# junyongeom/gru-mpi-cuda

Hardware: AMD Instinct MI355X
Metric: char-tokens/sec (whole node) for GRU hidden=512 at 1/2/4/8 MI355X (higher is better)
Workload: dtype bf16; 1 GPU; model=GRU L=1 H=512 E=512 V=256, global_batch=256, seq_len=32, parallelism=dp1, impl=hip, optimizer=adam, overlap=False, plan=fwd=persistent bwd0=persistent+dWhh+dP head=fwd-tail serial dP=bwd-tail, dp_plan=replicated, dp_pipeline=0, collectives=0

## Files before the change

### gru_mpi_cuda_amd/csrc/bindings.cpp

```cpp
#include <pybind11/pybind11.h>
#include <pybind11/numpy.h>
#include <pybind11/stl.h>

#include "engine/trainer.h"
#include "engine/generator.h"
#include "comm/rccl_comm.h"
#include "comm/bootstrap.h"
#include "data/name_loader.h"

namespace py = pybind11;
using namespace gk;

static hipStream_t S(uintptr_t s) { return reinterpret_cast<hipStream_t>(s); }
template <class T> static T* Pp(uintptr_t p) { return reinterpret_cast<T*>(p); }

template <class T>
static T get(const py::dict& d, const char* k, T dflt) {
  if (!d.contains(k)) return dflt;
  return d[k].cast<T>();
}
#define GP(T, d, k) reinterpret_cast<T*>(get<uintptr_t>(d, k, 0))

static OptimArgs optim_from(const py::dict& d, const std::string& who) {
  OptimArgs a;
// ... 367 lines not shown
  m.def("adam_step", [](py::dict o, uintptr_t s) {
    const OptimArgs a = optim_from(o, "adam_step");
    if (!a.g) throw std::runtime_error("adam_step: g required");
    adam_step(a, S(s));
    HIP_LAUNCH_CHECK();
  });
  m.def("grad_clip_scale", [](py::dict d, uintptr_t s) {
    const float* x = GP(const float, d, "x");
    float* parts = GP(float, d, "parts");
    float* scale = GP(float, d, "scale");
    const long n = get<long>(d, "n", 0);
    const int nparts = get<int>(d, "nparts", 0);
    if (!x || !parts || !scale || n < 0 || nparts < 1 || nparts > 4096)
      throw std::runtime_error("grad_clip_scale: x, parts, scale, n >= 0 and 1 <= nparts <= 4096 required");
    sumsq_partials(x, n, parts, nparts, S(s));
    HIP_LAUNCH_CHECK();
    clip_scale_finalize(parts, nparts, get<float>(d, "clip", 0.f), scale, S(s));
    HIP_LAUNCH_CHECK();
  });
  m.def("reduce_slabs_multi", [](py::list jobs, uintptr_t bump, uintptr_t s) {
    SlabJobs j;
    if (jobs.size() > 24) throw std::runtime_error("reduce_slabs_multi: at most 24 jobs");
    if (jobs.size() == 0) throw std::runtime_error("reduce_slabs_multi: no jobs");
    for (auto h : jobs) {
      py::dict d = h.cast<py::dict>();
      const float* src = GP(const float, d, "src");
      const int splits = get<int>(d, "splits", 1);
      if (!src || splits < 1) throw std::runtime_error("reduce_slabs_multi: src and splits >= 1 required");
      if (d.contains("bf") || d.contains("bfT") || d.contains("R") || d.contains("C")) {
        const int R = get<int>(d, "R", 0), C = get<int>(d, "C", 0);
        if (!GP(u16, d, "bf") && !GP(u16, d, "bfT")) throw std::runtime_error("reduce_slabs_multi: cast job needs bf or bfT");
        if (R <= 0 || C <= 0) throw std::runtime_error("reduce_slabs_multi: cast job needs R, C > 0");
        j.add_cast(src, splits, R, C, GP(float, d, "dst"), GP(u16, d, "bf"), GP(u16, d, "bfT"));
      } else {
        const long n = get<long>(d, "n", 0);
        if (n < 1 || !GP(float, d, "dst")) throw std::runtime_error("reduce_slabs_multi: plain job needs n >= 1 and dst");
        j.add(src, splits, n, GP(float, d, "dst"));
      }
    }
    j.bump = Pp<int>(bump);
    reduce_slabs_multi(j, S(s));
    HIP_LAUNCH_CHECK();
  });
  m.def("sum_partials", [](uintptr_t parts, int n, uintptr_t out, uintptr_t bump, uintptr_t s) {
    if (!parts || !out || n < 0) throw std::runtime_error("sum_partials: parts, out and n >= 0 required");
    sum_partials(Pp<const float>(parts), n, Pp<float>(out), S(s), Pp<int>(bump));
    HIP_LAUNCH_CHECK();
  });
  m.def("flat_pack_u32", [](uintptr_t p, uintptr_t pack, std::vector<std::pair<long, long>> ranges, long lo, long hi,
                            long tail, int unpack, uintptr_t s) {
    if (ranges.size() > 16) throw std::runtime_error("flat_pack_u32: at most 16 ranges");
    if (!p || !pack) throw std::runtime_error("flat_pack_u32: p and pack required");
    FlatRanges r;
    for (const auto& [off, n] : ranges) {
      if (off < 0 || n < 0 || n > (1L << 30)) throw std::runtime_error("flat_pack_u32: bad range");
      r.off[r.cnt] = off;
      r.n[r.cnt++] = (int)n;
    }
    flat_pack_u32(Pp<float>(p), Pp<unsigned>(pack), r, lo, hi, tail, unpack, S(s));
    HIP_LAUNCH_CHECK();
  });
  auto fwd_step_args = [](py::dict d) {
    FwdStepArgs a;
    a.hprev_bf = GP(const u16, d, "hprev_bf"); a.hprev_f = GP(const float, d, "hprev_f");
    a.Whh = GP(const u16, d, "Whh"); a.bhh = GP(const float, d, "bhh");
    a.P = GP(const float, d, "P"); a.ids = GP(const int, d, "ids"); a.Gi = GP(const float, d, "Gi");
    a.x_bf = GP(const u16, d, "x_bf"); a.Wih = GP(const u16, d, "Wih"); a.bih = GP(const float, d, "bih");
    a.Kin = get<int>(d, "Kin", 0);
    a.h_f = GP(float, d, "h_f"); a.h_bf = GP(u16, d, "h_bf"); a.hT = GP(u16, d, "hT");
    a.ldT = get<int>(d, "ldT", 0); a.colT = get<int>(d, "colT", 0);
    a.sr = GP(float, d, "sr"); a.sz = GP(float, d, "sz"); a.sn = GP(float, d, "sn"); a.sghn = GP(float, d, "sghn");
    a.s16 = GP(u16, d, "s16");
    a.Bp = get<int>(d, "Bp", 0); a.H = get<int>(d, "H", 0); a.algo = get<int>(d, "algo", 0);
    if (a.Bp % 32 || a.H % 64) throw std::runtime_error("fwd_step: Bp % 32 and H % 64 required");
    return a;
  };
  auto bwd_step_args = [](py::dict d) {
    BwdStepArgs a;
    a.dgh_next = GP(const u16, d, "dgh_next"); a.WhhT = GP(const u16, d, "WhhT");
    a.carry_in = GP(const float, d, "carry_in"); a.dy = GP(const float, d, "dy");
    a.r = GP(const float, d, "r"); a.z = GP(const float, d, "z"); a.n = GP(const float, d, "n");
    a.ghn = GP(const float, d, "ghn"); a.hprev = GP(const float, d, "hprev");
    a.carry_out = GP(float, d, "carry_out"); a.dgh = GP(u16, d, "dgh"); a.dghT = GP(u16, d, "dghT");
    a.dgiT = GP(u16, d, "dgiT"); a.dgi = GP(u16, d, "dgi");
    a.ldT = get<int>(d, "ldT", 0); a.colT = get<int>(d, "colT", 0);
    a.Bp = get<int>(d, "Bp", 0); a.H = get<int>(d, "H", 0); a.algo = get<int>(d, "algo", 0);
    a.sk_part = GP(float, d, "sk_part"); a.sk_part_floats = get<long>(d, "sk_part_floats", 0);
    a.sk_cnt = GP(unsigned, d, "sk_cnt"); a.sk_cnt_words = get<long>(d, "sk_cnt_words", 0);
    a.err = GP(unsigned, d, "err");
    a.dgiT_n_only = get<int>(d, "dgiT_n_only", 0);
    if (a.Bp % 32 || a.H % 64) throw std::runtime_error("bwd_step: Bp % 32 and H % 64 required");
    return a;
  };
  m.def("fwd_step", [fwd_step_args](py::dict d, uintptr_t s) {
    gru_fwd_step(fwd_step_args(d), S(s));
    HIP_LAUNCH_CHECK();
  });
  m.def("bwd_step", [bwd_step_args](py::dict d, uintptr_t s) {
    gru_bwd_step(bwd_step_args(d), S(s));
    HIP_LAUNCH_CHECK();
  });
  auto plan_dict = [](const StepPlan& p) {
    py::dict o;
    o["name"] = step_kernel_name(p.kernel);
    o["ks"] = p.ks; o["kb"] = p.kb; o["nks_i"] = p.nks_i; o["splits"] = p.splits; o["sk_map"] = p.sk_map;
    return o;
  };
  m.def("fwd_step_variant", [fwd_step_args, plan_dict](py::dict d) { return plan_dict(gru_fwd_step_plan(fwd_step_args(d))); });
  m.def("bwd_step_variant", [bwd_step_args, plan_dict](py::dict d) { return plan_dict(gru_bwd_step_plan(bwd_step_args(d))); });
  m.def("spin_delay", [](int us, uintptr_t s) { spin_delay(us, S(s)); HIP_LAUNCH_CHECK(); });
  m.def("copy_d2d", [](uintptr_t dst, uintptr_t src, size_t bytes) {
    HIP_CHECK(hipMemcpy(reinterpret_cast<void*>(dst), reinterpret_cast<const void*>(src), bytes, hipMemcpyDeviceToDevice));
  });
  m.def("graph_node_probe_detail", &graph_node_probe_detail);
  m.def("graph_node_probe", &graph_node_probe);
  m.def("block_cus", [](int nblocks, int us, uintptr_t s) { block_cus(nblocks, us, S(s)); });
  m.def("xcc_census", [](uintptr_t out, int nblocks, int threads, uintptr_t s) {
    xcc_census(Pp<unsigned>(out), nblocks, threads, S(s)); HIP_LAUNCH_CHECK(); });
  m.def("fwd_seq_supported", &gru_fwd_seq_supported);
  m.def("bwd_step_sk_splits", &gru_bwd_step_sk_splits);
  m.def("step_lds_variants", []() {
    const StepLdsVariants& v = step_lds_variants();
    py::dict d;
    d["fwd64"] = v.fwd64; d["bwd_sk_min_h"] = v.bwd_sk_min_h; d["dwfc_group"] = v.dwfc_group;
    d["bwd_big"] = v.bwd_big; d["bwd16"] = v.bwd16; d["bwd_xring"] = v.bwd_xring; d["fwd_xring"] = v.fwd_xring; d["fwd_fc"] = v.fwd_fc; d["fc_flash"] = v.fc_flash; d["fc_tail"] = v.fc_tail; d["bwd_tail"] = v.bwd_tail; d["save16"] = v.save16; d["big_dy"] = v.big_dy; d["ld_pad"] = v.ld_pad;
    return d;
  });
  m.def("set_step_lds_variants", [](py::dict d) {
    StepLdsVariants& v = step_lds_variants();
    for (auto kv : d) {
      const std::string k = py::str(kv.first);
      const int x = kv.second.cast<int>();
      if (k == "fwd64") v.fwd64 = x;
      else if (k == "bwd_sk_min_h") v.bwd_sk_min_h = x;
      else if (k == "dwfc_group") v.dwfc_group = x;
      else if (k == "bwd_big") v.bwd_big = x;
      else if (k == "bwd16") v.bwd16 = x;
      else if (k == "bwd_xring") v.bwd_xring = x;
      else if (k == "fwd_xring") v.fwd_xring = x;
      else if (k == "fwd_fc") v.fwd_fc = x;
      else if (k == "fc_flash") v.fc_flash = x;
      else if (k == "fc_tail") v.fc_tail = x;
      else if (k == "bwd_tail") v.bwd_tail = x;
      else if (k == "big_dy") v.big_dy = x;
      else if (k == "ld_pad") v.ld_pad = x;
      else if (k == "save16") v.save16 = x;
      else throw std::runtime_error("set_step_lds_variants: unknown field " + k);
    }
  });
  m.def("gemm_variants", []() {
    const GemmVariants& v = gemm_variants();
    py::dict d;
    d["mfma"] = v.mfma; d["phased"] = v.phased; d["sched"] = v.sched; d["groupm"] = v.groupm; d["onehot"] = v.onehot;
    return d;
  });
  m.def("set_gemm_variants", [](py::dict d) {
    GemmVariants& v = gemm_variants();
    for (auto kv : d) {
      const std::string k = py::str(kv.first);
      const int x = kv.second.cast<int>();
      if (k == "mfma") v.mfma = x;
      else if (k == "phased") v.phased = x;
      else if (k == "sched") v.sched = x;
      else if (k == "groupm") v.groupm = x;
      else if (k == "onehot") v.onehot = x;
      else throw std::runtime_error("set_gemm_variants: unknown field " + k);
    }
  });
  m.def("bwd_seq_supported", &gru_bwd_seq_supported);
  m.def("fwd_seq2", [](py::dict lo, py::dict hi, uintptr_t Wih, uintptr_t bih, uintptr_t s) {
    auto parse = [](py::dict d) {
      SeqFwdArgs a;
      a.HSb = GP(u16, d, "HSb"); a.HSf = GP(float, d, "HSf"); a.HT = GP(u16, d, "HT"); a.ldT = get<int>(d, "ldT", 0);
      a.HF = GP(u16, d, "HF"); a.xch = GP(u16, d, "xch");
      a.sr = GP(float, d, "sr"); a.sz = GP(float, d, "sz"); a.sn = GP(float, d, "sn"); a.sghn = GP(float, d, "sghn");
      a.Whh = GP(const u16, d, "Whh"); a.bhh = GP(const float, d, "bhh");
      a.P = GP(const float, d, "P"); a.ids = GP(const int, d, "ids"); a.Gi = GP(const float, d, "Gi");
      a.h0 = GP(const float, d, "h0");
      a.cnt = GP(unsigned, d, "cnt"); a.err = GP(unsigned, d, "err");
      a.dbg = GP(unsigned long long, d, "dbg"); a.allow_local = get<int>(d, "allow_local", 1);
      a.xring = get<int>(d, "xring", 0);
      a.s16 = GP(u16, d, "s16");
      a.zero_next = GP(unsigned, d, "zero_next"); a.zero_words = get<long>(d, "zero_words", 0);
      a.T = get<int>(d, "T", 0); a.Bp = get<int>(d, "Bp", 0); a.H = get<int>(d, "H", 0);
      if (!a.xch || !a.cnt || !a.HSb || !a.HSf || !a.Whh || !a.bhh) throw std::runtime_error("fwd_seq2: HSb/HSf/xch/cnt/Whh/bhh required");
      return a;
    };
    SeqFwd2Args a;
    a.lo = parse(lo); a.hi = parse(hi);
    a.Wih = reinterpret_cast<const u16*>(Wih); a.bih = reinterpret_cast<const float*>(bih);
    if (!a.lo.ids == !a.lo.Gi) throw std::runtime_error("fwd_seq2: lo needs exactly one of P+ids / Gi");
    if (!gru_fwd_seq2_supported(a.lo.H, a.lo.Bp)) throw std::runtime_error("fwd_seq2: shape not supported");
    gru_fwd_seq2(a, S(s));
    HIP_LAUNCH_CHECK();
  });
  m.def("fwd_seq2_supported", &gru_fwd_seq2_supported);
  m.def("fwd_seq_fc_supported", &gru_fwd_seq_fc_supported);
  m.def("fwd_seq_fc", [](py::dict d, py::dict fd, uintptr_t s) {
    SeqFwdArgs a;
    a.HSb = GP(u16, d, "HSb"); a.HSf = GP(float, d, "HSf"); a.HT = GP(u16, d, "HT"); a.ldT = get<int>(d, "ldT", 0);
    a.HF = GP(u16, d, "HF"); a.xch = GP(u16, d, "xch");
    a.sr = GP(float, d, "sr"); a.sz = GP(float, d, "sz"); a.sn = GP(float, d, "sn"); a.sghn = GP(float, d, "sghn");
    a.Whh = GP(const u16, d, "Whh"); a.bhh = GP(const float, d, "bhh");
    a.P = GP(const float, d, "P"); a.ids = GP(const int, d, "ids"); a.Gi = GP(const float, d, "Gi");
    a.h0 = GP(const float, d, "h0");
    a.cnt = GP(unsigned, d, "cnt"); a.err = GP(unsigned, d, "err");
    a.dbg = GP(unsigned long long, d, "dbg"); a.allow_local = get<int>(d, "allow_local", 1);
    a.xring = get<int>(d, "xring", 0);
    a.T = get<int>(d, "T", 0); a.Bp = get<int>(d, "Bp", 0); a.H = get<int>(d, "H", 0);
    SeqFcArgs f;
    f.Wf = GP(const u16, fd, "Wf"); f.WTf = GP(const u16, fd, "WTf"); f.b = GP(const float, fd, "b");
    f.labels = GP(const int, fd, "labels"); f.inv_count = GP(const float, fd, "inv_count");
    f.dy = GP(float, fd, "dy"); f.dlF = GP(u16, fd, "dlF"); f.loss_part = GP(float, fd, "loss_part");
    f.dW = GP(float, fd, "dW"); f.db = GP(float, fd, "db"); f.V = get<int>(fd, "V", 0);
    f.probe = get<int>(fd, "probe", 0);
    if (!a.xch || !a.cnt || !a.HSb || !a.HSf || !a.Whh || !a.bhh) throw std::runtime_error("fwd_seq_fc: HSb/HSf/xch/cnt/Whh/bhh required");
    if (!gru_fwd_seq_fc_supported(a.H, a.Bp, f.V)) throw std::runtime_error("fwd_seq_fc: shape not supported");
    gru_fwd_seq_fc(a, f, S(s));
    HIP_LAUNCH_CHECK();
  });
  m.def("fwd_seq", [](py::dict d, uintptr_t s) {
    SeqFwdArgs a;
    a.HSb = GP(u16, d, "HSb"); a.HSf = GP(float, d, "HSf"); a.HT = GP(u16, d, "HT"); a.ldT = get<int>(d, "ldT", 0);
    a.HF = GP(u16, d, "HF");
    a.xch = GP(u16, d, "xch");
    if (!a.xch) throw std::runtime_error("fwd_seq: exchange buffer xch [T][Bp][H] bf16 required");
    a.sr = GP(float, d, "sr"); a.sz = GP(float, d, "sz"); a.sn = GP(float, d, "sn"); a.sghn = GP(float, d, "sghn");
    a.Whh = GP(const u16, d, "Whh"); a.bhh = GP(const float, d, "bhh");
    a.P = GP(const float, d, "P"); a.ids = GP(const int, d, "ids"); a.Gi = GP(const float, d, "Gi");
    a.h0 = GP(const float, d, "h0");
    a.cnt = GP(unsigned, d, "cnt"); a.err = GP(unsigned, d, "err");
    a.dbg = GP(unsigned long long, d, "dbg"); a.allow_local = get<int>(d, "allow_local", 1);
    a.xring = get<int>(d, "xring", 0);
    a.s16 = GP(u16, d, "s16");
    a.zero_next = GP(unsigned, d, "zero_next"); a.zero_words = get<long>(d, "zero_words", 0);
    a.T = get<int>(d, "T", 0); a.Bp = get<int>(d, "Bp", 0); a.H = get<int>(d, "H", 0);
    if (!gru_fwd_seq_supported(a.H, a.Bp)) throw std::runtime_error("fwd_seq: shape not supported");
    gru_fwd_seq(a, S(s));
    HIP_LAUNCH_CHECK();
  });
  m.def("bwd_seq_big_supported", &gru_bwd_seq_big_supported);
  m.def("bwd_seq_big_part_floats", &gru_bwd_seq_big_part_floats);
  m.def("bwd_seq16_supported", &gru_bwd_seq16_supported);
  m.def("seq_flag_words", &seq_flag_words);
  m.def("bwd_seq", [](py::dict d, uintptr_t s) {
    SeqBwdArgs a;
    a.dy = GP(const float, d, "dy");
    a.sr = GP(const float, d, "sr"); a.sz = GP(const float, d, "sz"); a.sn = GP(const float, d, "sn");
    a.sghn = GP(const float, d, "sghn"); a.HSf = GP(const float, d, "HSf");
    a.HT = GP(const u16, d, "HT"); a.ldT = get<int>(d, "ldT", 0); a.WhhT = GP(const u16, d, "WhhT");
    a.HF = GP(const u16, d, "HF");
    a.xbuf = GP(u16, d, "xbuf"); a.dghT = GP(u16, d, "dghT"); a.dgiT = GP(u16, d, "dgiT");
    a.ldG = get<int>(d, "ldG", 0); a.dgi = GP(u16, d, "dgi");
    a.dWhh_part = GP(float, d, "dWhh_part"); a.dbhh_part = GP(float, d, "dbhh_part");
    a.dbih_part = GP(float, d, "dbih_part"); a.ids = GP(const int, d, "ids");
    a.dP_part = GP(float, d, "dP_part"); a.V = get<int>(d, "V", 0);
    a.cnt = GP(unsigned, d, "cnt"); a.err = GP(unsigned, d, "err"); a.dbg = GP(unsigned long long, d, "dbg");
    a.allow_local = get<int>(d, "allow_local", 1); a.xring = get<int>(d, "xring", 0);
    a.s16 = GP(const u16, d, "s16"); a.part = GP(float, d, "part");
    a.dl = GP(const u16, d, "dl"); a.WfcT = GP(const u16, d, "WfcT");
    a.dgiT_n_only = get<int>(d, "dgiT_n_only", 0);
    a.zero_next = GP(unsigned, d, "zero_next"); a.zero_words = get<long>(d, "zero_words", 0);
    a.T = get<int>(d, "T", 0); a.Bp = get<int>(d, "Bp", 0); a.H = get<int>(d, "H", 0);
    if (get<int>(d, "big", 0)) {
      gru_bwd_seq_big(a, S(s));
      HIP_LAUNCH_CHECK();
      return;
    }
    if (get<int>(d, "rows16", 0)) {
      if (!gru_bwd_seq16_supported(a.H, a.Bp, a.dP_part != nullptr)) throw std::runtime_error("bwd_seq(rows16): shape not supported");
      gru_bwd_seq16(a, S(s));
      HIP_LAUNCH_CHECK();
      return;
    }
    if (!get<int>(d, "unchecked", 0) &&
        !gru_bwd_seq_supported(a.H, a.Bp, a.dWhh_part != nullptr, a.dP_part != nullptr))
      throw std::runtime_error("bwd_seq: shape not supported");
    gru_bwd_seq(a, S(s));
    HIP_LAUNCH_CHECK();
  });
  auto fc_xent_args = [](const py::dict& d) {
    FcXentArgs a;
    a.X = GP(const u16, d, "X"); a.W = GP(const u16, d, "W"); a.b = GP(const float, d, "b");
    a.labels = GP(const int, d, "labels"); a.inv_count = GP(const float, d, "inv_count");
    a.dl = GP(u16, d, "dl"); a.dlT = GP(u16, d, "dlT"); a.loss_part = GP(float, d, "loss_part");
    a.M = get<int>(d, "M", 0); a.H = get<int>(d, "H", 0); a.V = get<int>(d, "V", 0);
    a.ldT = get<int>(d, "ldT", 0); a.colT = get<int>(d, "colT", 0);
    a.WT = GP(const u16, d, "WT"); a.dy = GP(float, d, "dy");
    a.dbg = GP(unsigned long long, d, "dbg");
    a.Wf = GP(const u16, d, "Wf"); a.WTf = GP(const u16, d, "WTf");
    return a;
  };
  m.def("fc_xent", [fc_xent_args](py::dict d, uintptr_t s) {
    const FcXentArgs a = fc_xent_args(d);
    if (a.M % 32 || a.V % 64 || a.V > 512 || a.H % 32 || a.ldT % 8 || a.colT % 8)
      throw std::runtime_error("fc_xent: bad shape");
    fc_xent(a, S(s));
    HIP_LAUNCH_CHECK();
  });
  m.def("fwd_seq_tail_supported", &gru_fwd_seq_tail_supported);
  m.def("fwd_seq_tail", [fc_xent_args](py::dict d, py::dict fd, uintptr_t s) {
    SeqFwdArgs a;
    a.HSb = GP(u16, d, "HSb"); a.HSf = GP(float, d, "HSf"); a.HT = GP(u16, d, "HT"); a.ldT = get<int>(d, "ldT", 0);
    a.HF = GP(u16, d, "HF"); a.xch = GP(u16, d, "xch");
    a.sr = GP(float, d, "sr"); a.sz = GP(float, d, "sz"); a.sn = GP(float, d, "sn"); a.sghn = GP(float, d, "sghn");
    a.Whh = GP(const u16, d, "Whh"); a.bhh = GP(const float, d, "bhh");
    a.P = GP(const float, d, "P"); a.ids = GP(const int, d, "ids"); a.Gi = GP(const float, d, "Gi");
    a.h0 = GP(const float, d, "h0");
    a.cnt = GP(unsigned, d, "cnt"); a.err = GP(unsigned, d, "err");
    a.dbg = GP(unsigned long long, d, "dbg"); a.allow_local = get<int>(d, "allow_local", 1);
    a.xring = get<int>(d, "xring", 0);
    a.s16 = GP(u16, d, "s16");
    a.zero_next = GP(unsigned, d, "zero_next"); a.zero_words = get<long>(d, "zero_words", 0);
    a.T = get<int>(d, "T", 0); a.Bp = get<int>(d, "Bp", 0); a.H = get<int>(d, "H", 0);
    const FcXentArgs f = fc_xent_args(fd);
    if (!a.xch || !a.cnt || !a.HSb || !a.HSf || !a.Whh || !a.bhh) throw std::runtime_error("fwd_seq_tail: HSb/HSf/xch/cnt/Whh/bhh required");
    if (!gru_fwd_seq_tail_supported(a.H, a.Bp, f.V)) throw std::runtime_error("fwd_seq_tail: shape not supported");
    gru_fwd_seq_tail(a, f, S(s));
// ... 284 lines not shown
```

### gru_mpi_cuda_amd/csrc/kernels/gemm_small.hip

```cpp
#include <algorithm>
#include <stdexcept>
#include <string>
#include "kernels.h"
#include "common.h"

namespace gk {

typedef __attribute__((address_space(3))) void lds_void_s;

DEV int xcd_remap_s(int orig, int nwg) {
  const int q = nwg / 8, r = nwg % 8, xcd = orig % 8;
  return (xcd < r ? xcd * (q + 1) : r * (q + 1) + (xcd - r) * q) + orig / 8;
}

template <int NKB, bool BIAS, bool ROWSUM>
DEV void gemm_small_body(const GemmArgs& a, int id, int ntn, int ntm, u16 (*lds)[2][64 * 64], int nch = 1) {
  const int tn = id % ntn, tm = (id / ntn) % ntm, sp = id / (ntn * ntm);
  const int lane = threadIdx.x & 63, w = threadIdx.x >> 6;
  const int wm = w >> 1, wn = w & 1;
  const int lr = lane & 15, lq = lane >> 4;
  const int row0 = tm * 64, col0 = tn * 64;
  const int srow = lane >> 3, sslot = lane & 7;

  f32x4 acc[2][2];
#pragma unroll
  for (int i = 0; i < 2; ++i)
#pragma unroll
    for (int j = 0; j < 2; ++j) acc[i][j] = f32x4{0.f, 0.f, 0.f, 0.f};
  const bool do_rs = ROWSUM && a.rowsumA && tn == 0 && wn == 0;
  float rs[2] = {0.f, 0.f};
  for (int ch = 0; ch < nch; ++ch) {
  const int kbeg = (sp * nch + ch) * NKB * 64;
  if (ch) __syncthreads();
#pragma unroll
  for (int kb = 0; kb < NKB; ++kb)
#pragma unroll
    for (int q = 0; q < 2; ++q) {
      const int r = w * 16 + q * 8 + srow;
      const int c = sslot ^ ((r >> 1) & 7);
      const size_t ko = (size_t)kbeg + kb * 64 + c * 8;
      if (!a.A32)
        __builtin_amdgcn_global_load_lds(a.A + (size_t)(row0 + r) * a.lda + ko,
                                         (lds_void_s*)(&lds[kb][0][(w * 16 + q * 8) * 64]), 16, 0, 0);
      __builtin_amdgcn_global_load_lds(a.B + (size_t)(col0 + r) * a.ldb + ko,
                                       (lds_void_s*)(&lds[kb][1][(w * 16 + q * 8) * 64]), 16, 0, 0);
    }
  if (a.A32) {
    const int tid = threadIdx.x;
#pragma unroll
    for (int kb = 0; kb < NKB; ++kb)
#pragma unroll
      for (int p = 0; p < 4; ++p) {
        const int q = tid + 256 * p;
        if (!a.a32_trans) {
          const int r = q >> 4, k4 = (q & 15) * 4;
          const float4 v = *reinterpret_cast<const float4*>(a.A32 + (size_t)(row0 + r) * a.lda + kbeg + kb * 64 + k4);
          const int c = (k4 >> 3) ^ ((r >> 1) & 7);
          uint2 u;
          u.x = (unsigned)f2bf(v.x) | ((unsigned)f2bf(v.y) << 16);
          u.y = (unsigned)f2bf(v.z) | ((unsigned)f2bf(v.w) << 16);
          *reinterpret_cast<uint2*>(&lds[kb][0][r * 64 + c * 8 + (k4 & 7)]) = u;
        } else {
          const int k = q >> 4, m4 = (q & 15) * 4;
          const float4 v = *reinterpret_cast<const float4*>(a.A32 + (size_t)(kbeg + kb * 64 + k) * a.lda + row0 + m4);
          const float e[4] = {v.x, v.y, v.z, v.w};
#pragma unroll
          for (int i = 0; i < 4; ++i) {
            const int r = m4 + i, c = (k >> 3) ^ ((r >> 1) & 7);
            lds[kb][0][r * 64 + c * 8 + (k & 7)] = f2bf(e[i]);
          }
        }
      }
  }
  asm volatile("s_waitcnt vmcnt(0)" ::: "memory");
  __syncthreads();

#pragma unroll
  for (int kb = 0; kb < NKB; ++kb)
#pragma unroll
    for (int ks = 0; ks < 2; ++ks) {
      const int c = ks * 4 + lq;
      bf16x8 af[2], bfr[2];
#pragma unroll
      for (int t = 0; t < 2; ++t) {
        const int ra = wm * 32 + t * 16 + lr, rb = wn * 32 + t * 16 + lr;
        af[t] = *reinterpret_cast<const bf16x8*>(&lds[kb][0][ra * 64 + ((c ^ ((ra >> 1) & 7)) * 8)]);
        bfr[t] = *reinterpret_cast<const bf16x8*>(&lds[kb][1][rb * 64 + ((c ^ ((rb >> 1) & 7)) * 8)]);
      }
#pragma unroll
      for (int i = 0; i < 2; ++i)
#pragma unroll
        for (int j = 0; j < 2; ++j) acc[i][j] = mfma16(af[i], bfr[j], acc[i][j]);
      if (do_rs) {
#pragma unroll
        for (int t = 0; t < 2; ++t)
#pragma unroll
          for (int e = 0; e < 8; ++e) rs[t] += (float)af[t][e];
      }
    }
  }

  float* C = a.C + (size_t)sp * a.M * a.ldc;
#pragma unroll
  for (int j = 0; j < 2; ++j) {
    const int col = col0 + wn * 32 + j * 16 + lr;
    const float bb = BIAS ? a.bias[col] : 0.f;
#pragma unroll
    for (int i = 0; i < 2; ++i)
#pragma unroll
      for (int e = 0; e < 4; ++e) {
        const int row = row0 + wm * 32 + i * 16 + lq * 4 + e;
        float* dst = C + (size_t)row * a.ldc + col;
        const float v = acc[i][j][e] + bb;
        if (a.accumulate) *dst += v; else *dst = v;
      }
  }
  if (do_rs) {
#pragma unroll
    for (int t = 0; t < 2; ++t) {
      float v = rs[t];
      v += __shfl_xor(v, 16, 64);
      v += __shfl_xor(v, 32, 64);
      if (lane < 16) a.rowsumA[(size_t)sp * a.M + row0 + wm * 32 + t * 16 + lane] = v;
    }
  }
}

template <int NKB, bool BIAS, bool ROWSUM>
__global__ void __launch_bounds__(256, NKB <= 4 ? 2 : 1) gemm_small_kernel(GemmArgs a, int ntn, int ntm, int nch) {
  __shared__ __attribute__((aligned(16))) u16 lds[NKB][2][64 * 64];
  gemm_small_body<NKB, BIAS, ROWSUM>(a, xcd_remap_s(blockIdx.x, gridDim.x), ntn, ntm, lds, nch);
}

struct SmallGroup { GemmArgs job[4]; int start[5], xs[5]; int ntn[4], ntm[4], nch[4]; int n, per_xcd; };

template <int NKB, bool BIAS, bool ROWSUM>
__global__ void __launch_bounds__(256, NKB <= 4 ? 2 : 1) gemm_small_group_kernel(SmallGroup g) {
  __shared__ __attribute__((aligned(16))) u16 lds[NKB][2][64 * 64];
  int k = 0, id;
  if (g.per_xcd) {
    const int x = blockIdx.x % 8, loc = blockIdx.x / 8;
    while (k + 1 < g.n && loc >= g.xs[k + 1]) ++k;
    id = x * (g.xs[k + 1] - g.xs[k]) + (loc - g.xs[k]);
  } else {
    const int gid = xcd_remap_s(blockIdx.x, gridDim.x);
    while (k + 1 < g.n && gid >= g.start[k + 1]) ++k;
    id = gid - g.start[k];
  }
  gemm_small_body<NKB, BIAS, ROWSUM>(g.job[k], id, g.ntn[k], g.ntm[k], lds, g.nch[k]);
}

template <int NKB, bool BIAS>
__global__ void __launch_bounds__(256, NKB <= 4 ? 2 : 1) gemm_small_prep_kernel(GemmArgs a, int ntn, int ntm,
                                                                                   PrepJob pj, int nprep, int nch) {
  __shared__ __attribute__((aligned(16))) u16 lds[NKB][2][64 * 64];
  const int ng = ntn * ntm * a.splits;
  if ((int)blockIdx.x >= ng) {
    prep_batch_body(pj, (int)blockIdx.x - ng, nprep);
    return;
  }
  gemm_small_body<NKB, BIAS, false>(a, xcd_remap_s(blockIdx.x, ng), ntn, ntm, lds, nch);
}

static int small_blocks(const GemmArgs& a, int* nch) {
  *nch = 1;
  if (a.onehot_ids || a.M % 64 || a.N % 64 || a.K % a.splits) return 0;
  const int kper = a.K / a.splits;
  if (kper % 64) return 0;
  int nkb = kper / 64;
  if (nkb > 8 && nkb % 8 == 0 && nkb <= 32) { *nch = nkb / 8; nkb = 8; }
  if (nkb != 2 && nkb != 3 && nkb != 4 && nkb != 8) return 0;
  if ((a.lda % 8) || (a.ldb % 8)) return 0;
  if ((reinterpret_cast<uintptr_t>(a.A32 ? (const void*)a.A32 : (const void*)a.A) |
       reinterpret_cast<uintptr_t>(a.B)) & 15) return 0;
  return nkb;
}
int gemm_small_kblocks(const GemmArgs& a) {
  int nch = 1;
  const int nkb = small_blocks(a, &nch);
  return nkb * nch;
}

template <class Launch>
static void dispatch_nkb(int nkb, bool bias, bool rs, const Launch& L) {
#define GS_CASE(N)                                                      \
  case N:                                                               \
    if (rs) { if (bias) L.template go<N, true, true>(); else L.template go<N, false, true>(); } \
    else { if (bias) L.template go<N, true, false>(); else L.template go<N, false, false>(); } \
    return;
  switch (nkb) { GS_CASE(2) GS_CASE(3) GS_CASE(4) GS_CASE(8) default: break; }
#undef GS_CASE
  throw std::runtime_error("gemm_small: unsupported K-slice");
}

struct SmallLaunch {
  const GemmArgs& a; int ntn, ntm, nch; hipStream_t s;
  template <int N, bool B, bool R> void go() const {
    hipLaunchKernelGGL((gemm_small_kernel<N, B, R>), dim3(ntn * ntm * a.splits), dim3(256), 0, s, a, ntn, ntm, nch);
  }
};
struct SmallGroupLaunch {
  const SmallGroup& g; int tot; hipStream_t s;
  template <int N, bool B, bool R> void go() const {
    hipLaunchKernelGGL((gemm_small_group_kernel<N, B, R>), dim3(tot), dim3(256), 0, s, g);
  }
};

void gemm_small(const GemmArgs& a, hipStream_t s) {
  int nch = 1;
  const int nkb = small_blocks(a, &nch);
  if (!nkb) throw std::runtime_error("gemm_small: unsupported shape");
  dispatch_nkb(nkb, a.bias && a.splits == 1, a.rowsumA != nullptr, SmallLaunch{a, a.N / 64, a.M / 64, nch, s});
}

void gemm_small_with_prep(const GemmArgs& a, const PrepJob& p, hipStream_t s) {
  int nch = 1;
  const int nkb = small_blocks(a, &nch);
  if (!nkb || a.rowsumA) throw std::runtime_error("gemm_small_with_prep: unsupported shape");
  const int ntn = a.N / 64, ntm = a.M / 64, nprep = prep_batch_blocks(p.T, p.Bp);
  int nkb2 = nkb;
  if (nkb == 8 && ntn * ntm * a.splits > 256) { nkb2 = 4; nch *= 2; }
  const dim3 grid(ntn * ntm * a.splits + nprep), block(256);
  const bool bias = a.bias && a.splits == 1;
#define GP_CASE(N)                                                                                        \
  case N:                                                                                                 \
    if (bias) hipLaunchKernelGGL((gemm_small_prep_kernel<N, true>), grid, block, 0, s, a, ntn, ntm, p, nprep, nch); \
    else hipLaunchKernelGGL((gemm_small_prep_kernel<N, false>), grid, block, 0, s, a, ntn, ntm, p, nprep, nch);     \
    return;
  switch (nkb2) { GP_CASE(2) GP_CASE(3) GP_CASE(4) GP_CASE(8) default: break; }
#undef GP_CASE
}

int gemm_small_group_depth(const GemmArgs* jobs, int n) {
  int nkb = 0;
  for (int k = 0; k < n; ++k) {
    const int kb = gemm_small_kblocks(jobs[k]);
    if (!kb) return 0;
    nkb = k ? std::min(nkb, kb) : kb;
  }
  while (nkb > 8) nkb = nkb % 8 ? 0 : 8;
  if (nkb != 2 && nkb != 3 && nkb != 4 && nkb != 8) return 0;
  for (int k = 0; k < n; ++k)
    if (gemm_small_kblocks(jobs[k]) % nkb) return 0;
  return nkb;
}

void gemm_small_group(const GemmArgs* jobs, int n, hipStream_t s) {
  if (n < 1 || n > 4) throw std::runtime_error("gemm_small_group: 1..4 jobs");
  SmallGroup g;
  g.n = n;
  int tot = 0;
  const int nkb = gemm_small_group_depth(jobs, n);
  const bool bias = jobs[0].bias && jobs[0].splits == 1;
  bool rs = false;
  g.per_xcd = 1;
  g.xs[0] = 0;
  for (int k = 0; k < n; ++k) {
    const GemmArgs& a = jobs[k];
    if (!nkb || (a.bias && a.splits == 1) != bias)
      throw std::runtime_error("gemm_small_group: job " + std::to_string(k) + " incompatible");
    rs = rs || a.rowsumA != nullptr;
    g.job[k] = a;
    g.ntn[k] = a.N / 64; g.ntm[k] = a.M / 64;
    g.nch[k] = gemm_small_kblocks(a) / nkb;
    g.start[k] = tot;
    const int nt = g.ntn[k] * g.ntm[k] * a.splits;
    tot += nt;
    if (nt % 8) g.per_xcd = 0;
    g.xs[k + 1] = g.xs[k] + nt / 8;
  }
  g.start[n] = tot;
  dispatch_nkb(nkb, bias, rs, SmallGroupLaunch{g, tot, s});
}

}
```

### gru_mpi_cuda_amd/csrc/kernels/kernels.h

```cpp
#pragma once
#include <vector>
#include <hip/hip_runtime.h>
#include <stdint.h>

typedef unsigned short u16;
#define DEV_HOST_INLINE __host__ __device__ __forceinline__

namespace gk {

struct FwdStepArgs {
  const u16* hprev_bf = nullptr;
  const float* hprev_f = nullptr;
  const u16* Whh = nullptr;
  const float* bhh = nullptr;
  const float* P = nullptr;
  const int* ids = nullptr;
  const float* Gi = nullptr;
  const u16* x_bf = nullptr;
  const u16* Wih = nullptr;
  const float* bih = nullptr;
  int Kin = 0;
  float* h_f = nullptr;
  u16* h_bf = nullptr;
  u16* hT = nullptr;
  int ldT = 0, colT = 0;
  float* sr = nullptr; float* sz = nullptr; float* sn = nullptr; float* sghn = nullptr;
  u16* s16 = nullptr;
  int Bp = 0, H = 0;
  int algo = 0;
};
void gru_fwd_step(const FwdStepArgs& a, hipStream_t s);

struct BwdStepArgs {
  int dgiT_n_only = 0;
  const u16* dgh_next = nullptr;
  const u16* WhhT = nullptr;
  const float* carry_in = nullptr;
  const float* dy = nullptr;
  const float *r = nullptr, *z = nullptr, *n = nullptr, *ghn = nullptr;
  const float* hprev = nullptr;
  float* carry_out = nullptr;
  u16* dgh = nullptr;
  u16* dghT = nullptr;
  u16* dgiT = nullptr;
  u16* dgi = nullptr;
  int ldT = 0, colT = 0, Bp = 0, H = 0;
  int algo = 0;
  float* sk_part = nullptr;
  long sk_part_floats = 0;
  unsigned* sk_cnt = nullptr;
  long sk_cnt_words = 0;
  int sk_map = 0;
  unsigned* err = nullptr;
};
void gru_bwd_step(const BwdStepArgs& a, hipStream_t s);
int gru_bwd_step_sk_splits(int H, int Bp);
struct StepLdsVariants {
  int fwd64 = 1;
  int bwd_sk_min_h = 1024;
  int dwfc_group = 1;
  int bwd_big = 1;
  int bwd16 = 1;
  int bwd_xring = 2;
  int fwd_xring = 4;
  int save16 = 1;
  int fc_flash = 0;
  int fwd_fc = 0;
  int fc_tail = 1;
  int bwd_tail = 1;
  int big_dy = 1;
  int ld_pad = -1;
};
StepLdsVariants& step_lds_variants();
struct GemmVariants {
  int mfma = 0;
  int phased = -1;
  int sched = -1;
  int groupm = 4;
  int onehot = 1;
};
GemmVariants& gemm_variants();
bool gru_step_lds_ok(int H, int Bp);
bool gru_step_picks_lds(int algo, int H, int Bp);
void gru_fwd_step_lds(const FwdStepArgs& a, hipStream_t s);
void gru_bwd_step_lds(const BwdStepArgs& a, hipStream_t s);
enum StepKernel { kStepReg = 0, kStepLds128, kStepLds64, kStepBig, kStepLds8, kStepSk2, kStepSk4 };
struct StepPlan { int kernel = kStepReg; int ks = 0, kb = 0, nks_i = 0; int splits = 0, sk_map = 0; };
const char* step_kernel_name(int kernel);
StepPlan gru_fwd_step_plan(const FwdStepArgs& a);
StepPlan gru_bwd_step_plan(const BwdStepArgs& a);
StepPlan gru_fwd_step_lds_plan(const FwdStepArgs& a);
StepPlan gru_bwd_step_lds_plan(const BwdStepArgs& a);

struct PrepJob { const int* in = nullptr; int Bmax = 0, T = 0, Bp = 0; int* ids = nullptr; int* labels = nullptr; float* inv_count = nullptr; };
struct SeqFwdArgs {
  u16* HSb = nullptr;
  u16* xch = nullptr;
  float* HSf = nullptr;
  u16* HT = nullptr; int ldT = 0;
  u16* HF = nullptr;
  float *sr = nullptr, *sz = nullptr, *sn = nullptr, *sghn = nullptr;
  u16* s16 = nullptr;
  const u16* Whh = nullptr; const float* bhh = nullptr;
  const float* P = nullptr; const int* ids = nullptr;
  const float* Gi = nullptr;
  const float* h0 = nullptr;
  unsigned* cnt = nullptr;
  unsigned* zero_next = nullptr;
  long zero_words = 0;
  unsigned* err = nullptr;
  unsigned long long* dbg = nullptr;
  int allow_local = 1;
  int xring = 0;
  int T = 0, Bp = 0, H = 0;
};
static constexpr int kFcCons = 32;
inline long seq_flag_words(int H, int Bp) { return (long)(Bp / 32) * (H / 16 + kFcCons) * 16; }
bool gru_fwd_seq_supported(int H, int Bp);
void gru_fwd_seq(const SeqFwdArgs& a, hipStream_t s);
struct SeqFcArgs {
  const u16* Wf = nullptr;
  const u16* WTf = nullptr;
  const float* b = nullptr;
  const int* labels = nullptr;
  const float* inv_count = nullptr;
  float* dy = nullptr;
  u16* dlF = nullptr;
  float* loss_part = nullptr;
  float* dW = nullptr;
  float* db = nullptr;
  int V = 0;
  int probe = 0;
};
bool gru_fwd_seq_fc_supported(int H, int Bp, int V);
void gru_fwd_seq_fc(const SeqFwdArgs& a, const SeqFcArgs& f, hipStream_t s);
struct FcXentArgs;
bool gru_fwd_seq_tail_supported(int H, int Bp, int V);
void gru_fwd_seq_tail(const SeqFwdArgs& a, const FcXentArgs& f, hipStream_t s);


struct SeqFwd2Args {
  SeqFwdArgs lo, hi;
  const u16* Wih = nullptr;
  const float* bih = nullptr;
};
bool gru_fwd_seq2_supported(int H, int Bp);
void gru_fwd_seq2(const SeqFwd2Args& a, hipStream_t s);

struct SeqBwdArgs {
  const float* dy = nullptr;
  const float *sr = nullptr, *sz = nullptr, *sn = nullptr, *sghn = nullptr;
  const u16* s16 = nullptr;
  const float* HSf = nullptr;
  const u16* HT = nullptr; int ldT = 0;
  const u16* HF = nullptr;
  const u16* WhhT = nullptr;
  u16* xbuf = nullptr;
  u16* dghT = nullptr; u16* dgiT = nullptr; int ldG = 0;
  u16* dgi = nullptr;
  float* dWhh_part = nullptr;
  float* dbhh_part = nullptr;
  float* dbih_part = nullptr;
  const int* ids = nullptr;
  float* dP_part = nullptr; int V = 0;
  unsigned* cnt = nullptr;
  unsigned* zero_next = nullptr;
  long zero_words = 0;
  unsigned* err = nullptr;
  unsigned long long* dbg = nullptr;
  int allow_local = 1;
  float* part = nullptr;
  int dgiT_n_only = 0;
  const u16* dl = nullptr;
  const u16* WfcT = nullptr;
  int xring = 0;
  int T = 0, Bp = 0, H = 0;
};
bool gru_bwd_seq_supported(int H, int Bp, bool fuse_w, bool fuse_p);
void gru_bwd_seq(const SeqBwdArgs& a, hipStream_t s);
struct BwdTailArgs {
  u16* dP_bf = nullptr;
  u16* dPT_bf = nullptr;
  const float* loss_part = nullptr; int nloss = 0;
  float* loss = nullptr;
  int* step = nullptr;
};
bool gru_bwd_seq_tail_supported(int H, int Bp, int V);
void gru_bwd_seq_tail(const SeqBwdArgs& a, const BwdTailArgs& t, hipStream_t s);
bool gru_bwd_seq16_supported(int H, int Bp, bool fuse_p);
void gru_bwd_seq16(const SeqBwdArgs& a, hipStream_t s);
bool gru_bwd_seq_big_supported(int H, int Bp);
long gru_bwd_seq_big_part_floats(int H, int Bp);
void gru_bwd_seq_big(const SeqBwdArgs& a, hipStream_t s);

struct FcXentArgs {
  const u16* X = nullptr;
  const u16* W = nullptr;
  const float* b = nullptr;
  const int* labels = nullptr;
  const float* inv_count = nullptr;
  u16* dl = nullptr;
  u16* dlT = nullptr;
  float* loss_part = nullptr;
  const u16* WT = nullptr;
  float* dy = nullptr;
  int M = 0, H = 0, V = 0, ldT = 0, colT = 0;
  const u16* Wf = nullptr;
  const u16* WTf = nullptr;
  unsigned long long* dbg = nullptr;
};
void fc_xent(const FcXentArgs& a, hipStream_t s);
void softmax_xent(const float* logits, const FcXentArgs& a, hipStream_t s);
bool fc_xent_fused_ok(int V, int H, int M);

struct FcSampleArgs {
  const u16* X = nullptr;
  const u16* W = nullptr;
  const u16* Wf = nullptr;
  const float* b = nullptr;
  const float* rf = nullptr;
  int* ids = nullptr;
  unsigned char* out = nullptr;
  int* alive = nullptr;
  float* probs = nullptr;
  int N = 0, Bp = 0, H = 0, V = 0, step = 0, max_len = 0, eos = 0;
};
void fc_sample(const FcSampleArgs& a, hipStream_t s);

struct GemmF32Args {
  const float* A = nullptr; int lda = 0;
  const float* B = nullptr; int ldb = 0;
  float* C = nullptr; int ldc = 0;
// ... 283 lines not shown
```

Measured before the change: 42.74 million char-tokens/s.

## Add multi-slot LDS ring pipeline for small GEMM kernels

Adds a ring-buffered variant of the small GEMM with 3 or 4 LDS slots. Async global-to-LDS loads are issued several K-blocks ahead, and waits use vmcnt counts, replacing the old scheme that staged all K-blocks (or chunks of them) up front. The variant is enabled by default with 4 slots for the plain, grouped and prep-fused GEMM paths. It should overlap memory latency with MFMA work and cap LDS use independent of K. The cost is a barrier per K-block and a different occupancy profile.

```diff
diff --git a/gru_mpi_cuda_amd/csrc/bindings.cpp b/gru_mpi_cuda_amd/csrc/bindings.cpp
--- a/gru_mpi_cuda_amd/csrc/bindings.cpp
+++ b/gru_mpi_cuda_amd/csrc/bindings.cpp
@@ -543,6 +543,7 @@
     const GemmVariants& v = gemm_variants();
     py::dict d;
     d["mfma"] = v.mfma; d["phased"] = v.phased; d["sched"] = v.sched; d["groupm"] = v.groupm; d["onehot"] = v.onehot;
+    d["small_ring"] = v.small_ring;
     return d;
   });
   m.def("set_gemm_variants", [](py::dict d) {
@@ -555,6 +556,10 @@
       else if (k == "sched") v.sched = x;
       else if (k == "groupm") v.groupm = x;
       else if (k == "onehot") v.onehot = x;
+      else if (k == "small_ring") {
+        if (x != 0 && x != 3 && x != 4) throw std::runtime_error("set_gemm_variants: small_ring is 0, 3 or 4");
+        v.small_ring = x;
+      }
       else throw std::runtime_error("set_gemm_variants: unknown field " + k);
     }
   });
diff --git a/gru_mpi_cuda_amd/csrc/kernels/gemm_small.hip b/gru_mpi_cuda_amd/csrc/kernels/gemm_small.hip
--- a/gru_mpi_cuda_amd/csrc/kernels/gemm_small.hip
+++ b/gru_mpi_cuda_amd/csrc/kernels/gemm_small.hip
@@ -126,6 +126,157 @@
   }
 }
 
+typedef __attribute__((address_space(3))) const void* gs_lds_cptr;
+typedef unsigned gs_u32x4 __attribute__((ext_vector_type(4)));
+DEV gs_u32x4 gs_rd128(const u16* p) {
+  gs_u32x4 v;
+  asm volatile("ds_read_b128 %0, %1" : "=v"(v) : "v"((gs_lds_cptr)p) : "memory");
+  return v;
+}
+template <int N> DEV void gs_vm_wait() { asm volatile("s_waitcnt vmcnt(%0)" ::"n"(N) : "memory"); }
+template <int A> DEV void gs_wait_ahead(int ahead) {
+  if (ahead >= A) { gs_vm_wait<4 * A>(); return; }
+  if constexpr (A > 0) gs_wait_ahead<A - 1>(ahead);
+}
+
+template <int S, bool BIAS, bool ROWSUM>
+DEV void gemm_small_ring_body(const GemmArgs& a, int id, int ntn, int ntm, int nk, u16* r0, u16* r1, u16* r2, u16* r3) {
+  static_assert(S == 3 || S == 4, "ring of 3 or 4 slots");
+  const int tn = id % ntn, tm = (id / ntn) % ntm, sp = id / (ntn * ntm);
+  const int lane = threadIdx.x & 63, w = threadIdx.x >> 6;
+  const int wm = w >> 1, wn = w & 1;
+  const int lr = lane & 15, lq = lane >> 4;
+  const int row0 = tm * 64, col0 = tn * 64;
+  const int srow = lane >> 3, sslot = lane & 7;
+
+  const u16 *srcA[2], *srcB[2];
+#pragma unroll
+  for (int q = 0; q < 2; ++q) {
+    const int r = w * 16 + q * 8 + srow;
+    const int c = sslot ^ ((r >> 1) & 7);
+    const size_t ko = (size_t)sp * nk * 64 + c * 8;
+    srcA[q] = a.A + (size_t)(row0 + r) * a.lda + ko;
+    srcB[q] = a.B + (size_t)(col0 + r) * a.ldb + ko;
+  }
+  auto stage = [&](u16* slot, int kb) {
+#pragma unroll
+    for (int q = 0; q < 2; ++q) {
+      __builtin_amdgcn_global_load_lds(srcA[q] + kb * 64, (lds_void_s*)(&slot[(w * 16 + q * 8) * 64]), 16, 0, 0);
+      __builtin_amdgcn_global_load_lds(srcB[q] + kb * 64, (lds_void_s*)(&slot[64 * 64 + (w * 16 + q * 8) * 64]), 16, 0, 0);
+    }
+  };
+#pragma unroll
+  for (int s = 0; s < S - 1; ++s)
+    if (s < nk) stage(s == 0 ? r0 : s == 1 ? r1 : r2, s);
+
+  f32x4 acc[2][2];
+#pragma unroll
+  for (int i = 0; i < 2; ++i)
+#pragma unroll
+    for (int j = 0; j < 2; ++j) acc[i][j] = f32x4{0.f, 0.f, 0.f, 0.f};
+  const bool do_rs = ROWSUM && a.rowsumA && tn == 0 && wn == 0;
+  float rs[2] = {0.f, 0.f};
+
+  int oa[2][2], ob[2][2];
+#pragma unroll
+  for (int ks = 0; ks < 2; ++ks)
+#pragma unroll
+    for (int t = 0; t < 2; ++t) {
+      const int c = ks * 4 + lq;
+      const int ra = wm * 32 + t * 16 + lr, rb = wn * 32 + t * 16 + lr;
+      oa[ks][t] = ra * 64 + ((c ^ ((ra >> 1) & 7)) * 8);
+      ob[ks][t] = 64 * 64 + rb * 64 + ((c ^ ((rb >> 1) & 7)) * 8);
+    }
+
+  auto block = [&](const u16* R, u16* N, int kb) {
+    gs_wait_ahead<S - 2>(min(S - 2, nk - 1 - kb));
+    lds_barrier();
+    if (kb + S - 1 < nk) stage(N, kb + S - 1);
+    gs_u32x4 ua[2][2], ub[2][2];
+#pragma unroll
+    for (int ks = 0; ks < 2; ++ks)
+#pragma unroll
+      for (int t = 0; t < 2; ++t) {
+        ua[ks][t] = gs_rd128(R + oa[ks][t]);
+        ub[ks][t] = gs_rd128(R + ob[ks][t]);
+      }
+    asm volatile("s_waitcnt lgkmcnt(0)" ::: "memory");
+    bf16x8 af[2][2], bfr[2][2];
+#pragma unroll
+    for (int ks = 0; ks < 2; ++ks)
+#pragma unroll
+      for (int t = 0; t < 2; ++t) {
+        asm volatile("" : "+v"(ua[ks][t]), "+v"(ub[ks][t]));
+        af[ks][t] = __builtin_bit_cast(bf16x8, ua[ks][t]);
+        bfr[ks][t] = __builtin_bit_cast(bf16x8, ub[ks][t]);
+      }
+#pragma unroll
+    for (int ks = 0; ks < 2; ++ks) {
+#pragma unroll
+      for (int i = 0; i < 2; ++i)
+#pragma unroll
+        for (int j = 0; j < 2; ++j) acc[i][j] = mfma16(af[ks][i], bfr[ks][j], acc[i][j]);
+      if (do_rs) {
+#pragma unroll
+        for (int t = 0; t < 2; ++t)
+#pragma unroll
+          for (int e = 0; e < 8; ++e) rs[t] += (float)af[ks][t][e];
+      }
+    }
+  };
+  if constexpr (S == 4) {
+    for (int kb = 0; kb < nk; kb += 4) {
+      block(r0, r3, kb);
+      if (kb + 1 < nk) block(r1, r0, kb + 1);
+      if (kb + 2 < nk) block(r2, r1, kb + 2);
+      if (kb + 3 < nk) block(r3, r2, kb + 3);
+    }
+  } else {
+    for (int kb = 0; kb < nk; kb += 3) {
+      block(r0, r2, kb);
+      if (kb + 1 < nk) block(r1, r0, kb + 1);
+      if (kb + 2 < nk) block(r2, r1, kb + 2);
+    }
+  }
+
+  float* C = a.C + (size_t)sp * a.M * a.ldc;
+#pragma unroll
+  for (int j = 0; j < 2; ++j) {
+    const int col = col0 + wn * 32 + j * 16 + lr;
+    const float bb = BIAS ? a.bias[col] : 0.f;
+#pragma unroll
+    for (int i = 0; i < 2; ++i)
+#pragma unroll
+      for (int e = 0; e < 4; ++e) {
+        const int row = row0 + wm * 32 + i * 16 + lq * 4 + e;
+        float* dst = C + (size_t)row * a.ldc + col;
+        const float v = acc[i][j][e] + bb;
+        if (a.accumulate) *dst += v; else *dst = v;
+      }
+  }
+  if (do_rs) {
+#pragma unroll
+    for (int t = 0; t < 2; ++t) {
+      float v = rs[t];
+      v += __shfl_xor(v, 16, 64);
+      v += __shfl_xor(v, 32, 64);
+      if (lane < 16) a.rowsumA[(size_t)sp * a.M + row0 + wm * 32 + t * 16 + lane] = v;
+    }
+  }
+}
+
+#define GS_RING_SLOTS(S)                                                  \
+  __shared__ __attribute__((aligned(16))) u16 r0[2 * 64 * 64];            \
+  __shared__ __attribute__((aligned(16))) u16 r1[2 * 64 * 64];            \
+  __shared__ __attribute__((aligned(16))) u16 r2[2 * 64 * 64];            \
+  __shared__ __attribute__((aligned(16))) u16 r3[S == 4 ? 2 * 64 * 64 : 8];
+
+template <int S, bool BIAS, bool ROWSUM>
+__global__ void __launch_bounds__(256, S == 3 ? 3 : 2) gemm_small_ring_kernel(GemmArgs a, int ntn, int ntm, int nk) {
+  GS_RING_SLOTS(S)
+  gemm_small_ring_body<S, BIAS, ROWSUM>(a, xcd_remap_s(blockIdx.x, gridDim.x), ntn, ntm, nk, r0, r1, r2, r3);
+}
+
 template <int NKB, bool BIAS, bool ROWSUM>
 __global__ void __launch_bounds__(256, NKB <= 4 ? 2 : 1) gemm_small_kernel(GemmArgs a, int ntn, int ntm, int nch) {
   __shared__ __attribute__((aligned(16))) u16 lds[NKB][2][64 * 64];
@@ -162,6 +313,54 @@
   gemm_small_body<NKB, BIAS, false>(a, xcd_remap_s(blockIdx.x, ng), ntn, ntm, lds, nch);
 }
 
+template <int S, bool BIAS, bool ROWSUM>
+__global__ void __launch_bounds__(256, S == 3 ? 3 : 2) gemm_small_ring_group_kernel(SmallGroup g) {
+  GS_RING_SLOTS(S)
+  int k = 0, id;
+  if (g.per_xcd) {
+    const int x = blockIdx.x % 8, loc = blockIdx.x / 8;
+    while (k + 1 < g.n && loc >= g.xs[k + 1]) ++k;
+    id = x * (g.xs[k + 1] - g.xs[k]) + (loc - g.xs[k]);
+  } else {
+    const int gid = xcd_remap_s(blockIdx.x, gridDim.x);
+    while (k + 1 < g.n && gid >= g.start[k + 1]) ++k;
+    id = gid - g.start[k];
+  }
+  gemm_small_ring_body<S, BIAS, ROWSUM>(g.job[k], id, g.ntn[k], g.ntm[k], g.nch[k], r0, r1, r2, r3);
+}
+
+template <int S, bool BIAS>
+__global__ void __launch_bounds__(256, S == 3 ? 3 : 2) gemm_small_ring_prep_kernel(GemmArgs a, int ntn, int ntm, PrepJob pj,
+                                                                                    int nprep, int nk) {
+  GS_RING_SLOTS(S)
+  const int ng = ntn * ntm * a.splits;
+  if ((int)blockIdx.x >= ng) {
+    prep_batch_body(pj, (int)blockIdx.x - ng, nprep);
+    return;
+  }
+  gemm_small_ring_body<S, BIAS, false>(a, xcd_remap_s(blockIdx.x, ng), ntn, ntm, nk, r0, r1, r2, r3);
+}
+
+static int ring_slots(const GemmArgs* jobs, int n) {
+  const int v = gemm_variants().small_ring;
+  if (v == 0) return 0;
+  if (v != 3 && v != 4) throw std::runtime_error("gemm_small: small_ring is 0, 3 or 4");
+  for (int k = 0; k < n; ++k)
+    if (jobs[k].A32) return 0;
+  return v;
+}
+
+template <class Launch>
+static void dispatch_ring(int S, bool bias, bool rs, const Launch& L) {
+  if (S == 3) {
+    if (rs) { if (bias) L.template ring<3, true, true>(); else L.template ring<3, false, true>(); }
+    else { if (bias) L.template ring<3, true, false>(); else L.template ring<3, false, false>(); }
+  } else {
+    if (rs) { if (bias) L.template ring<4, true, true>(); else L.template ring<4, false, true>(); }
+    else { if (bias) L.template ring<4, true, false>(); else L.template ring<4, false, false>(); }
+  }
+}
+
 static int small_blocks(const GemmArgs& a, int* nch) {
   *nch = 1;
   if (a.onehot_ids || a.M % 64 || a.N % 64 || a.K % a.splits) return 0;
@@ -198,18 +397,28 @@
   template <int N, bool B, bool R> void go() const {
     hipLaunchKernelGGL((gemm_small_kernel<N, B, R>), dim3(ntn * ntm * a.splits), dim3(256), 0, s, a, ntn, ntm, nch);
   }
+  template <int S, bool B, bool R> void ring() const {
+    hipLaunchKernelGGL((gemm_small_ring_kernel<S, B, R>), dim3(ntn * ntm * a.splits), dim3(256), 0, s, a, ntn, ntm, nch);
+  }
 };
 struct SmallGroupLaunch {
   const SmallGroup& g; int tot; hipStream_t s;
   template <int N, bool B, bool R> void go() const {
     hipLaunchKernelGGL((gemm_small_group_kernel<N, B, R>), dim3(tot), dim3(256), 0, s, g);
   }
+  template <int S, bool B, bool R> void ring() const {
+    hipLaunchKernelGGL((gemm_small_ring_group_kernel<S, B, R>), dim3(tot), dim3(256), 0, s, g);
+  }
 };
 
 void gemm_small(const GemmArgs& a, hipStream_t s) {
   int nch = 1;
   const int nkb = small_blocks(a, &nch);
   if (!nkb) throw std::runtime_error("gemm_small: unsupported shape");
+  if (const int S = ring_slots(&a, 1)) {
+    dispatch_ring(S, a.bias && a.splits == 1, a.rowsumA != nullptr, SmallLaunch{a, a.N / 64, a.M / 64, nkb * nch, s});
+    return;
+  }
   dispatch_nkb(nkb, a.bias && a.splits == 1, a.rowsumA != nullptr, SmallLaunch{a, a.N / 64, a.M / 64, nch, s});
 }
 
@@ -218,10 +427,19 @@
   const int nkb = small_blocks(a, &nch);
   if (!nkb || a.rowsumA) throw std::runtime_error("gemm_small_with_prep: unsupported shape");
   const int ntn = a.N / 64, ntm = a.M / 64, nprep = prep_batch_blocks(p.T, p.Bp);
+  const dim3 grid(ntn * ntm * a.splits + nprep), block(256);
+  const bool bias = a.bias && a.splits == 1;
+  if (const int S = ring_slots(&a, 1)) {
+    const int nk = nkb * nch;
+#define GP_RING(S_)                                                                                                        \
+    if (bias) hipLaunchKernelGGL((gemm_small_ring_prep_kernel<S_, true>), grid, block, 0, s, a, ntn, ntm, p, nprep, nk);  \
+    else hipLaunchKernelGGL((gemm_small_ring_prep_kernel<S_, false>), grid, block, 0, s, a, ntn, ntm, p, nprep, nk);
+    if (S == 3) { GP_RING(3) } else { GP_RING(4) }
+#undef GP_RING
+    return;
+  }
   int nkb2 = nkb;
   if (nkb == 8 && ntn * ntm * a.splits > 256) { nkb2 = 4; nch *= 2; }
-  const dim3 grid(ntn * ntm * a.splits + nprep), block(256);
-  const bool bias = a.bias && a.splits == 1;
 #define GP_CASE(N)                                                                                        \
   case N:                                                                                                 \
     if (bias) hipLaunchKernelGGL((gemm_small_prep_kernel<N, true>), grid, block, 0, s, a, ntn, ntm, p, nprep, nch); \
@@ -270,6 +488,11 @@
     g.xs[k + 1] = g.xs[k] + nt / 8;
   }
   g.start[n] = tot;
+  if (const int S = ring_slots(jobs, n)) {
+    for (int k = 0; k < n; ++k) g.nch[k] *= nkb;
+    dispatch_ring(S, bias, rs, SmallGroupLaunch{g, tot, s});
+    return;
+  }
   dispatch_nkb(nkb, bias, rs, SmallGroupLaunch{g, tot, s});
 }
 
diff --git a/gru_mpi_cuda_amd/csrc/kernels/kernels.h b/gru_mpi_cuda_amd/csrc/kernels/kernels.h
--- a/gru_mpi_cuda_amd/csrc/kernels/kernels.h
+++ b/gru_mpi_cuda_amd/csrc/kernels/kernels.h
@@ -78,6 +78,7 @@
   int sched = -1;
   int groupm = 4;
   int onehot = 1;
+  int small_ring = 4;
 };
 GemmVariants& gemm_variants();
 bool gru_step_lds_ok(int H, int Bp);
```

Result: faster. 43.34 million char-tokens/s (median of 6 runs) (+1.4%).
